# theouterlimitz/Audio-Mastering-Engine

Measured on AMD Instinct MI355X. Metric: mastered Msamples/sec (48 kHz stereo f32) at 1/2/4/8 GPUs; % HBM roofline, higher is better.
Workload: dtype f64

## Files before the change

### audio-mastering-engine_amd/csrc/amx_chain.hip

```cpp
#include "amx_dev.hpp"


namespace amx {

#define AMX_HALF_LUT 32769

__device__ __forceinline__ void decode_in(const ChainDev &cd, const uint32_t *row, int f,
                                          int win, int16_t &l, int16_t &r) {
    if (win == 2) {
        l = q_f32_to_s16_ffmpeg(__uint_as_float(row[2 * f]));
        r = q_f32_to_s16_ffmpeg(__uint_as_float(row[2 * f + 1]));
    } else {
        const uint32_t w = row[f];
        if (cd.in_s16) {
            l = lo16(w);
            r = hi16(w);
        } else {
            l = r = q_f32_to_s16_ffmpeg(__uint_as_float(w));
        }
    }
}

template <int D, int WIN, bool AN, bool SC = false>
__global__ void __launch_bounds__(AMX_BLOCK) k_front1(const ChainDev *__restrict__ cdp,
// ... 335 lines not shown
#pragma unroll
                for (int e = 0; e < 2; e++) {
                    const int qq = (int)q_f32_to_s16_ffmpeg(src[e]);
                    const float v = s_tab[abs(qq)];
                    t2[e] = __int_as_float(__float_as_int(v) | (qq & (int)0x80000000));
                }
                int16_t l, rr;
                analog_shelves(cd, t2[0], t2[1], l, rr);
                a16[q.loc_off + fr] = pack2(l, rr);
            }
        }
    }
}

#define AMX_G16_PITCH (AMX_TF + 4)
template <int D>
__global__ void __launch_bounds__(AMX_BLOCK, 4) k_gemv16(const ChainDev *__restrict__ cdp,
                                                         const ChunkDev *__restrict__ chunks,
                                                         const SegDev *__restrict__ segs,
                                                         int n_seg, int L,
                                                         const uint32_t *__restrict__ a16,
                                                         const double *__restrict__ G,
                                                         double *__restrict__ e) {
    constexpr int ROWS = AMX_BLOCK / 2;
    constexpr int H = D / 2;
    constexpr int GQ = AMX_TF * D / 2;
    static_assert(GQ <= AMX_BLOCK && D % 2 == 0 && D > 0, "tile shape");
    __shared__ __attribute__((aligned(16))) uint32_t s_in[ROWS * AMX_G16_PITCH];
    __shared__ __attribute__((aligned(16))) double sG[AMX_TF * D];
    __shared__ int64_t rb[ROWS];
    __shared__ int rl[ROWS];
// ... 16 lines not shown
    }
    uint4 R[2], RG;
    auto fetch = [&](int k) {
        RG = *reinterpret_cast<const uint4 *>(G + (int64_t)k * D + 2 * (t < GQ ? t : 0));
#pragma unroll
        for (int m = 0; m < 2; m++) {
            const int n = k + c4;
            uint4 v = *reinterpret_cast<const uint4 *>(ip[m] + (n < ilen[m] ? k : 0));
            R[m] = v;
        }
    };
    double a0[H], a1[H];
#pragma unroll
    for (int d = 0; d < H; d++) { a0[d] = 0.0; a1[d] = 0.0; }
    fetch(0);
    const uint32_t *rp = s_in + row * AMX_G16_PITCH;
    for (int k = 0; k < L; k += AMX_TF) {
#pragma unroll
        for (int m = 0; m < 2; m++) {
            uint4 v = R[m];
            const int n = k + c4;
            v.x = n < ilen[m] ? v.x : 0u;
            v.y = n + 1 < ilen[m] ? v.y : 0u;
            v.z = n + 2 < ilen[m] ? v.z : 0u;
            v.w = n + 3 < ilen[m] ? v.w : 0u;
            *reinterpret_cast<uint4 *>(s_in + ((t >> 2) + 64 * m) * AMX_G16_PITCH + c4) = v;
        }
        if (t < GQ) reinterpret_cast<uint4 *>(sG)[t] = RG;
        __syncthreads();
        fetch(k + AMX_TF < L ? k + AMX_TF : k);
#pragma unroll 1
        for (int f = 0; f < AMX_TF; f++) {
            const uint32_t w = rp[f];
            const double x0 = (double)((float)lo16(w) / 32768.0f);
            const double x1 = (double)((float)hi16(w) / 32768.0f);
            const double *g = sG + f * D + half * H;
#pragma unroll
            for (int d = 0; d < H; d++) {
                a0[d] = fma(g[d], x0, a0[d]);
                a1[d] = fma(g[d], x1, a1[d]);
            }
        }
        __syncthreads();
    }
    if (valid && !sg.last) {
        double *eo = e + (int64_t)j * 2 * D + half * H;
#pragma unroll
        for (int d = 0; d < H; d++) { eo[d] = a0[d]; eo[D + d] = a1[d]; }
    }
}
// ... 52 lines not shown
        }
    }
}

__device__ __forceinline__ VRows vt_rows(int32_t base, int len) {
    VRows vr;
    const int r0 = (threadIdx.x & 63) >> 2;
#pragma unroll
    for (int i = 0; i < 2; i++) {
        vr.base[i] = __shfl(base, 2 * (r0 + 16 * i));
        vr.len[i] = __shfl(len, 2 * (r0 + 16 * i));
    }
    return vr;
}

template <int MASK, bool MB, bool KW, bool SC = false>
__global__ void __launch_bounds__(AMX_BLOCK, (MB || KW) ? 4 : 5) k_front2(const ChainDev *__restrict__ cdp,
                                                      const ChunkDev *__restrict__ chunks,
                                                      const SegDev *__restrict__ segs, int n_seg,
                                                      int L, const uint32_t *__restrict__ a16,
                                                      const double *__restrict__ s_eq,
                                                      uint32_t *__restrict__ dst, int to_out,
                                                      const double *__restrict__ Gx,
                                                      double *__restrict__ e_x,
                                                      const double *__restrict__ Gkw,
                                                      double *__restrict__ e_kw,
                                                      uint32_t *__restrict__ pk,
                                                      const float *__restrict__ slut) {
    constexpr int D = EqDim<MASK>::v;
    constexpr int ROWS = AMX_BLOCK / 2;
    constexpr int WV = AMX_BLOCK / 64;
// ... 22 lines not shown
            for (int d = 0; d < D; d++) z[d] = s[d];
        }
    }
    EqState est;
    eq_state_load<MASK>(est, z);
    double xv[MB ? AMX_XO_DIM : 1];
#pragma unroll
    for (int d = 0; d < (MB ? AMX_XO_DIM : 1); d++) xv[d] = 0.0;
    double kv[KW ? AMX_KW_DIM : 1];
#pragma unroll
    for (int d = 0; d < (KW ? AMX_KW_DIM : 1); d++) kv[d] = 0.0;
    int kmax = 0;
    const int klen = (j < n_seg) ? segs[j].len : 0;
    const int negm = (cd.st[0].neg ? 1 : 0) | (cd.st[3].neg ? 8 : 0);
    const float w = cd.width;
    const int won = cd.width_on;
    const VRows vin = vt_rows(b_in, len);
    if (chn == 0) s_orow[wv][row] = make_int2(b_out, len);
    uint32_t *s_in = s_in_all[wv], *s_out = s_out_all[wv];
    vt4 R[2];
    vt_fetch(R, a16, vin, 0);
    for (int k = 0; k < L; k += AMX_TF) {
        vt_put(s_in, R, vin, k);
        amx_wave_sync();
        vt_next(R, a16, vin, k, L);
        const uint32_t *rp = s_in + row * AMX_VT_PITCH;
        uint32_t *op = s_out + row * AMX_VT_PITCH;
#pragma unroll 1
        for (int f0 = 0; f0 < AMX_TF; f0 += AMX_EQ_F) {
            float xf[AMX_EQ_F];
            double x[AMX_EQ_F];
#pragma unroll
            for (int f = 0; f < AMX_EQ_F; f++) {
                const uint32_t p = rp[f0 + f];
                const int16_t sv = chn ? hi16(p) : lo16(p);
                if constexpr (SC) xf[f] = slut ? slut[(int)sv + 32768] : (float)sv / 32768.0f;
                else xf[f] = (float)sv / 32768.0f;
                x[f] = (double)xf[f];
            }
            eq_tile<MASK, AMX_EQ_F>(negm, cd.eqc + (f0 & cd.pad0_), est, x, xf);
#pragma unroll
            for (int f = 0; f < AMX_EQ_F; f++) {
                int16_t qv;
                if constexpr (SC) {
                    qv = MASK ? f64_to_s16(x[f]) : f32_to_s16(xf[f]);
                } else {
                    float v = MASK ? (float)x[f] : xf[f];
                    if (won) {
                        const float o = pair_swap(v);
                        v = width_one(w, chn ? o : v, chn ? v : o, chn);
                    }
                    qv = f32_to_s16(v);
                }
                const int other = __builtin_amdgcn_update_dpp(0, (int)qv, 0xB1, 0xF, 0xF, false);
                if (chn == 0) op[f0 + f] = pack2(qv, (int16_t)other);
                if constexpr (MB) {
                    const double *g = Gx + (int64_t)(k + f0 + f) * AMX_XO_DIM;
                    const double xd = (double)((float)qv / 32768.0f);
#pragma unroll
                    for (int d = 0; d < AMX_XO_DIM; d++) xv[d] = fma(g[d], xd, xv[d]);
                }
                if constexpr (KW) {
                    const int n = k + f0 + f;
                    const bool act = n < klen;
                    kmax = max(kmax, act ? abs((int)qv) : 0);
                    const double xs = act ? (double)qv * (1.0 / 32768.0) : 0.0;
                    const double *g = Gkw + (int64_t)n * AMX_KW_DIM;
#pragma unroll
                    for (int d = 0; d < AMX_KW_DIM; d++) kv[d] = fma(g[d], xs, kv[d]);
                }
            }
        }
        amx_wave_sync();
        {
            const int r0 = (t & 63) >> 2;
            const int2 o0 = s_orow[wv][r0], o1 = s_orow[wv][r0 + 16];
            VRows vout;
            vout.base[0] = o0.x; vout.len[0] = o0.y;
            vout.base[1] = o1.x; vout.len[1] = o1.y;
            vt_store(s_out, dst, vout, k);
        }
// ... 53 lines not shown
#pragma unroll
    for (int sc = 0; sc < 4; sc++) {
        c[5 * sc + 0] = s_c[6 * sc + 0];
        c[5 * sc + 1] = s_c[6 * sc + 1];
        c[5 * sc + 2] = s_c[6 * sc + 2];
        c[5 * sc + 3] = s_c[6 * sc + 4];
        c[5 * sc + 4] = s_c[6 * sc + 5];
    }
    uint32_t *si = s_in[wv], *slo = s_b[wv][0], *smi = s_b[wv][1], *shi = si;
    vt4 R[2];
    vt_fetch(R, p16, vr, 0);
    for (int k = 0; k < L; k += AMX_TF) {
        vt_put(si, R, vr, k);
        amx_wave_sync();
        vt_next(R, p16, vr, k, L);
        uint32_t xin[AMX_TF];
#pragma unroll
        for (int q = 0; q < AMX_TF / 4; q++) {
            const vt4 v = *reinterpret_cast<const vt4 *>(si + row * AMX_VT_PITCH + 4 * q);
            xin[4 * q] = v.x; xin[4 * q + 1] = v.y; xin[4 * q + 2] = v.z; xin[4 * q + 3] = v.w;
        }
        const int o = row * AMX_VT_PITCH;
#pragma unroll 4
        for (int f = 0; f < AMX_TF; f++) {
            const uint32_t p = xin[f];
            const int16_t v = chn ? hi16(p) : lo16(p);
            const double x = (double)((float)v / 32768.0f);
            double l = bq_step(c, z[0], z[1], x);
            l = bq_step(c + 5, z[2], z[3], l);
            double h = bq_step(c + 10, z[4], z[5], x);
            h = bq_step(c + 15, z[6], z[7], h);
            const double m = (x - l) - h;
            const int ql = f64_to_s16(l), qm = f64_to_s16(m), qh = f64_to_s16(h);
            const int ol = __builtin_amdgcn_update_dpp(0, ql, 0xB1, 0xF, 0xF, false);
            const int om = __builtin_amdgcn_update_dpp(0, qm, 0xB1, 0xF, 0xF, false);
            const int oh = __builtin_amdgcn_update_dpp(0, qh, 0xB1, 0xF, 0xF, false);
            if (chn == 0) {
                slo[o + f] = pack2((int16_t)ql, (int16_t)ol);
                smi[o + f] = pack2((int16_t)qm, (int16_t)om);
            } else {
                shi[o + f] = pack2((int16_t)oh, (int16_t)qh);
            }
        }
        amx_wave_sync();
        vt_store(slo, bands, vr, k);
        vt_store(smi, bands + nloc, vr, k);
        vt_store(shi, bands + 2 * nloc, vr, k);
        amx_wave_sync();
    }
}

template <int D, int WIN, bool AN, bool SC = false>
static hipError_t front1_t(const Launch &l, const uint32_t *in, const float *lut, uint32_t *a16,
                           const double *G, double *e) {
    hipLaunchKernelGGL((k_front1<D, WIN, AN, SC>), grid1(l.n_seg), dim3(AMX_BLOCK), 0, l.stream, l.cd,
                       l.chunks, l.segs, l.n_seg, l.L, in, lut, a16, G, e);
// ... 15 lines not shown
static hipError_t front1s_t(const Launch &l, const uint32_t *in, const float *lut, uint32_t *a16,
                            const double *G, double *e) {
    const int rows = AMX_BLOCK / 2;
    if constexpr (AN) {
        if (l.f1_mode == AMX_F1_SPLIT && l.lut_half) {
            const int64_t wgs = l.an_blocks;
            const dim3 gh((unsigned)(wgs < cu_count() ? (wgs > 0 ? wgs : 1) : cu_count()));
            const bool vec = l.an_vec && (reinterpret_cast<uintptr_t>(in) & 15) == 0;
            if (vec)
                hipLaunchKernelGGL(k_analog_h<true>, gh, dim3(1024), 0, l.stream, l.cd, l.chunks, l.n_chunks,
                                   reinterpret_cast<const float *>(in), l.lut_half, a16, l.an_blocks);
            else
                hipLaunchKernelGGL(k_analog_h<false>, gh, dim3(1024), 0, l.stream, l.cd, l.chunks, l.n_chunks,
                                   reinterpret_cast<const float *>(in), l.lut_half, a16, l.an_blocks);
            if constexpr (D > 0) {
                hipLaunchKernelGGL((k_gemv16<D>), dim3((unsigned)((l.n_seg + rows - 1) / rows)), dim3(AMX_BLOCK), 0,
                                   l.stream, l.cd, l.chunks, l.segs, l.n_seg, l.L, a16, G, e);
            }
            return hipGetLastError();
        }
    }
    dim3 grid((unsigned)((l.n_seg + rows - 1) / rows));
    hipLaunchKernelGGL((k_front1s<D, AN>), grid, dim3(AMX_BLOCK), 0, l.stream, l.cd, l.chunks,
                       l.segs, l.n_seg, l.L, in, lut, a16, G, e);
    return hipGetLastError();
}

template <int D, int WIN>
static hipError_t front1_an(const Launch &l, bool an, const uint32_t *in, const float *lut,
                            uint32_t *a16, const double *G, double *e) {
    if constexpr (WIN == 2) {
        if (l.L % AMX_TF) return hipErrorInvalidValue;
// ... 9 lines not shown
    if (l.n_seg <= 0) return hipSuccess;
    if (analog && !lut) return hipErrorInvalidValue;
    if (sc && (analog || win != 1)) return hipErrorInvalidValue;
    const uint32_t *i32 = reinterpret_cast<const uint32_t *>(in);
    uint32_t *a = reinterpret_cast<uint32_t *>(a16);
#define F1(DD)                                                                   \
    case DD:                                                                     \
        if (sc) return front1_t<DD, 1, false, true>(l, i32, lut, a, G, e);       \
        return win == 2 ? front1_an<DD, 2>(l, analog, i32, lut, a, G, e)         \
                        : front1_an<DD, 1>(l, analog, i32, lut, a, G, e);
    switch (D) { F1(0) F1(2) F1(4) F1(8) F1(10) F1(12) F1(16) F1(18) F1(20) }
#undef F1
    return hipErrorInvalidValue;
}

template <int MASK, bool MB, bool KW, bool SC = false>
static hipError_t front2_t(const Launch &l, const uint32_t *a16, const double *s_eq,
                           uint32_t *dst, int to_out, const double *Gx, double *e_x,
                           const double *Gkw, double *e_kw, uint32_t *pk, const float *slut = nullptr) {
    const int rows = AMX_BLOCK / 2;
    dim3 grid((unsigned)((l.n_seg + rows - 1) / rows));
    hipLaunchKernelGGL((k_front2<MASK, MB, KW, SC>), grid, dim3(AMX_BLOCK), 0, l.stream, l.cd,
                       l.chunks, l.segs, l.n_seg, l.L, a16, s_eq, dst, to_out, Gx, e_x, Gkw, e_kw,
                       pk, slut);
    return hipGetLastError();
}

#define AMX_MASK_CASES(X) X(0) X(1) X(2) X(3) X(4) X(5) X(6) X(7) X(8) X(9) X(10) X(11) X(12) X(13) X(14) X(15)

hipError_t launch_front2(const Launch &l, int mask, const int16_t *a16, const double *s_eq,
                         int16_t *dst, int to_out, const double *Gx, double *e_x,
                         const double *Gkw, double *e_kw, uint32_t *pk, bool sc, const float *slut) {
    if (l.n_seg <= 0) return hipSuccess;
    const uint32_t *a = reinterpret_cast<const uint32_t *>(a16);
    uint32_t *d = reinterpret_cast<uint32_t *>(dst);
    const bool mb = Gx != nullptr, kw = Gkw != nullptr;
    if (mb && kw) return hipErrorInvalidValue;
    if (sc && kw) return hipErrorInvalidValue;
    switch (mask) {
#define C2(M)                                                                           \
    case M:                                                                             \
        if (sc) return mb ? front2_t<M, true, false, true>(l, a, s_eq, d, to_out, Gx, e_x, Gkw, e_kw, pk, slut) \
                          : front2_t<M, false, false, true>(l, a, s_eq, d, to_out, Gx, e_x, Gkw, e_kw, pk, slut); \
        return mb ? front2_t<M, true, false>(l, a, s_eq, d, to_out, Gx, e_x, Gkw, e_kw, pk) \
             : kw ? front2_t<M, false, true>(l, a, s_eq, d, to_out, Gx, e_x, Gkw, e_kw, pk) \
                  : front2_t<M, false, false>(l, a, s_eq, d, to_out, Gx, e_x, Gkw, e_kw, pk);
        AMX_MASK_CASES(C2)
#undef C2
    }
    return hipErrorInvalidValue;
}

hipError_t launch_xover2(const Launch &l, const int16_t *p16, const double *s_x,
                         int16_t *bands, int64_t nloc, int *bact) {
    if (l.n_seg <= 0) return hipSuccess;
    const int rows = AMX_BLOCK / 2;
    dim3 grid((unsigned)((l.n_seg + rows - 1) / rows));
    hipLaunchKernelGGL(k_xover2, grid, dim3(AMX_BLOCK), 0, l.stream, l.cd, l.chunks, l.segs,
                       l.n_seg, l.L, reinterpret_cast<const uint32_t *>(p16), s_x,
// ... 6 lines not shown
```

### audio-mastering-engine_amd/csrc/amx_dev.hpp

```cpp
#pragma once
#include "amx_internal.hpp"
#include <math.h>

namespace amx {

__device__ __forceinline__ int16_t q_f32_to_s16_ffmpeg(float x) {
    float v = rintf(x * 32768.0f);
    v = fminf(fmaxf(v, -32768.0f), 32767.0f);
    return (int16_t)(int)v;
}
__device__ __forceinline__ int16_t f32_to_s16(float x) {
    const float v = __builtin_amdgcn_fmed3f(x, -1.0f, 1.0f) * 32767.0f;
    return (int16_t)(int)v;
}
__device__ __forceinline__ double f64_clip1_raw(double x);
__device__ __forceinline__ int16_t f64_to_s16(double x) {
    return (int16_t)(int)(f64_clip1_raw(x) * 32767.0);
}
__device__ __forceinline__ double round2(double v) {
    if (!isfinite(v)) return v;
    const double p = v * 100.0;
    const double err = fma(v, 100.0, -p);
    double k = rint(p);
    if (fabs(p - k) == 0.5 && err != 0.0) k = err > 0.0 ? floor(p) + 1.0 : floor(p);
    return k / 100.0;
}
__device__ __forceinline__ int16_t sat16(int v) {
    return (int16_t)(v > 32767 ? 32767 : (v < -32768 ? -32768 : v));
}
__device__ __forceinline__ uint32_t pack2(int16_t a, int16_t b) {
    return (uint32_t)(uint16_t)a | ((uint32_t)(uint16_t)b << 16);
}
// ... 131 lines not shown
#pragma unroll
        for (int i = 0; i < 8; i++) st.pa[i] = z[o + i];
        o += 8;
    }
    if constexpr ((MASK & 4) != 0) {
#pragma unroll
        for (int i = 0; i < 8; i++) {
            if constexpr ((MASK & 2) != 0) st.pb[i] = z[o + i];
            else st.pa[i] = z[o + i];
        }
        o += 8;
    }
    if constexpr ((MASK & 8) != 0) { st.s3[0] = z[o]; st.s3[1] = z[o + 1]; }
}

template <int MASK, int F>
__device__ __forceinline__ void eq_tile(int negm, const double *__restrict__ sq, EqState &st,
                                        double *x, const float *xf) {
    constexpr int NP = ((MASK >> 1) & 1) + ((MASK >> 2) & 1);
    int c = 0;
    if constexpr ((MASK & 1) != 0) {
        double q[6];
#pragma unroll
        for (int i = 0; i < 6; i++) q[i] = sq[i];
        if (!(negm & 1)) {
#pragma unroll
            for (int f = 0; f < F; f++) {
                const double y = bq_step(q, st.s0[0], st.s0[1], x[f]);
                x[f] = x[f] + (y - x[f]) * q[5];
            }
        } else {
#pragma unroll
            for (int f = 0; f < F; f++) {
                const double y = bq_step(q, st.s0[0], st.s0[1], x[f]);
                const double xg = (double)(xf[f] * (float)q[5]);
                x[f] = xg + (y - xg);
            }
        }
        c = 6;
    }
    if constexpr (NP > 0) {
#pragma unroll 1
        for (int sidx = 0; sidx < NP; sidx++) {
            const double *q = sq + c + 21 * sidx;
            double b[F];
#pragma unroll
            for (int f = 0; f < F; f++) b[f] = x[f];
#pragma unroll
            for (int k = 0; k < 4; k++)
#pragma unroll
                for (int f = 0; f < F; f++)
                    b[f] = bq_step(q + 5 * k, st.pa[2 * k], st.pa[2 * k + 1], b[f]);
            const double gm1 = q[20];
#pragma unroll
            for (int f = 0; f < F; f++) x[f] = x[f] + b[f] * gm1;
            if constexpr (NP == 2) {
#pragma unroll
                for (int i = 0; i < 8; i++) { const double tmp = st.pa[i]; st.pa[i] = st.pb[i]; st.pb[i] = tmp; }
            }
        }
        c += 21 * NP;
    }
    if constexpr ((MASK & 8) != 0) {
        double q[6];
#pragma unroll
        for (int i = 0; i < 6; i++) q[i] = sq[c + i];
        if (!(negm & 8)) {
#pragma unroll
            for (int f = 0; f < F; f++) {
                const double y = bq_step(q, st.s3[0], st.s3[1], x[f]);
                x[f] = x[f] + (y - x[f]) * q[5];
            }
        } else {
#pragma unroll
// ... 6 lines not shown
                    const double xg = x[f] * q[5];
                    x[f] = xg + (y - xg);
                }
            }
        }
    }
}

__device__ __forceinline__ void width_frame(float w, float &l, float &r) {
    float mid = (l + r) / 2.0f, side = (l - r) / 2.0f;
    side = side * w;
    float nl = mid + side, nr = mid - side;
    l = __builtin_amdgcn_fmed3f(nl, -1.0f, 1.0f);
    r = __builtin_amdgcn_fmed3f(nr, -1.0f, 1.0f);
}
__device__ __forceinline__ float width_one(float w, float l, float r, int chn) {
    const float mid = (l + r) / 2.0f, side = ((l - r) / 2.0f) * w;
    return __builtin_amdgcn_fmed3f(chn ? mid - side : mid + side, -1.0f, 1.0f);
}

#define AMX_TF AMX_TF_FRAMES
template <int W, int ROWS = AMX_BLOCK>
struct Tile {
    static constexpr int ROW = AMX_TF * W;
    static constexpr int PITCH = ROW + 1;
    static constexpr int WORDS = ROWS * PITCH;
    static constexpr int ITER = ROWS * ROW / AMX_BLOCK;
    static constexpr int RSTEP = AMX_BLOCK / ROW;
    static constexpr int RW = ROWS / (AMX_BLOCK / 64);
};

template <int W, int ROWS, bool LOCAL>
__device__ __forceinline__ int tile_row(int m) {
// ... 75 lines not shown
__device__ __forceinline__ void tile_store(const uint32_t *lds, uint32_t *__restrict__ dst,
                                           const int64_t *rb, const int *hi, int k) {
    using T = Tile<W, ROWS>;
    const int c = threadIdx.x % T::ROW;
    const int n = k + c / W;
#pragma unroll
    for (int m = 0; m < T::ITER; m++) {
        const int r = tile_row<W, ROWS, LOCAL>(m);
        if (n < hi[r]) dst[rb[r] + (int64_t)n * W + (c % W)] = lds[r * T::PITCH + c];
    }
}

__device__ __forceinline__ float pair_swap(float v) {
    return __int_as_float(__builtin_amdgcn_update_dpp(0, __float_as_int(v), 0xB1, 0xF, 0xF, false));
}
__device__ __forceinline__ double pair_swap(double v) {
    const int64_t b = __double_as_longlong(v);
    const int lo = __builtin_amdgcn_update_dpp(0, (int)(b & 0xffffffff), 0xB1, 0xF, 0xF, false);
    const int hi = __builtin_amdgcn_update_dpp(0, (int)(b >> 32), 0xB1, 0xF, 0xF, false);
    return __longlong_as_double(((int64_t)hi << 32) | (uint32_t)lo);
}

static inline dim3 grid1(int64_t n) { return dim3((unsigned)((n + AMX_BLOCK - 1) / AMX_BLOCK)); }
static inline bool empty(dim3 g) { return g.x == 0 || g.y == 0 || g.z == 0; }

}
```

### audio-mastering-engine_amd/csrc/amx_dyn.hip

```cpp
#include "amx_dev.hpp"

namespace amx {

typedef double d2v __attribute__((ext_vector_type(2)));
typedef uint32_t u4v __attribute__((ext_vector_type(4)));

#define AMX_TAB 32769

#define AMX_RMS_N 4096
#define AMX_RMS_MAXLOOK 1024

__device__ __forceinline__ int rms_slot(int k) { return k + (k >> 4); }

__device__ __forceinline__ uint32_t rms_floor(uint64_t S, uint32_t cnt, double rc) {
    const double sd = fma((double)(uint32_t)(S >> 32), 4294967296.0, (double)(uint32_t)S);
    const double cd = (double)cnt;
    const uint32_t k = (uint32_t)__builtin_amdgcn_sqrtf((float)(sd * rc));
    const uint32_t k1 = k + 1;
    const bool up = (double)__umul24(k1, k1) * cd <= sd;
    const bool down = (double)__umul24(k, k) * cd > sd;
    const uint32_t r = k + (uint32_t)up - (uint32_t)(down & !up);
    return cnt ? (r > 32768u ? 32768u : r) : 0u;
}

// ... 356 lines not shown
    const uint16_t *irow[4];
#pragma unroll
    for (int i = 0; i < 4; i++) {
        const int r = 16 * i + (lane >> 2);
        irow[i] = mi + __shfl(rowoff + start, r) + 4 * (lane & 3);
    }
    u2v I[AMX_ENV_PF][4];
#pragma unroll
    for (int u = 0; u < AMX_ENV_PF; u++)
#pragma unroll
        for (int i = 0; i < 4; i++) I[u][i] = *reinterpret_cast<const u2v *>(irow[i] + u * AMX_ENV_TF);
    double G[2][16];
    env_gather(mt, I[0], G[0]);
    env_gather(mt, I[1], G[1]);
    double att = 0.0, s_spec = 0.0;
    if (cd.env_guess && start >= 0) att = mt[mi[rowoff + start]];
    bool any = false;
    for (int q0 = 0; q0 < ntile; q0 += AMX_ENV_PF) {
#pragma unroll
        for (int u = 0; u < AMX_ENV_PF; u++)
            env0_tile<RCP>(cd, sm, G[u & 1], I[u], I[(u + 2) % AMX_ENV_PF], irow, mt,
                           q0 + u, ntile, nwarm, start, end, ckr, att, s_spec, any);
    }
    if (valid) {
        sv[(int64_t)b * ld + j] = s_spec;
        ev[(int64_t)b * ld + j] = att;
        act[(int64_t)b * ld + j] = any ? 1 : 0;
    }
}

template <bool RCP>
// ... 673 lines not shown
```

### audio-mastering-engine_amd/csrc/amx_internal.hpp

```cpp
#pragma once
#include <hip/hip_runtime.h>
#include <stdint.h>

#include "amx_tables.hpp"

#define AMX_BLOCK 256
#define AMX_HIST_BINS 1000
#define AMX_SCAN_PW 6
#define AMX_CTL_FAST 1
#define AMX_STATS 16
#ifndef AMX_PCM_U8
#define AMX_PCM_U8 0
#define AMX_PCM_S16 1
#define AMX_PCM_S24 2
#define AMX_PCM_S32 3
#define AMX_PCM_F32 4
#define AMX_PCM_F64 5
#define AMX_PCM_S8 6
#define AMX_PCM_S16BE 7
#define AMX_PCM_S24BE 8
#define AMX_PCM_S32BE 9
#define AMX_PCM_F32BE 10
#define AMX_PCM_F64BE 11
#endif

struct amx_flac_cand_t;

namespace amx {
struct Launch {
    const ChainDev *cd;
    const ChunkDev *chunks;
    const SegDev *segs;
    int32_t n_chunks, n_seg, L;
    hipStream_t stream;
    const float *lut_half = nullptr;
    int f1_mode = AMX_F1_SPLIT;
    int64_t max_chunk_n = 0;
    int64_t an_blocks = 0;
    int an_vec = 0;
};
struct ScanPlan {
    int D, n_blk, K;
    const ScanBlk *blks;
    const double *M;
    const double *Mbk;
};
hipError_t launch_front1(const Launch &l, int D, int win, bool analog, const float *in,
                         const float *lut, int16_t *a16, const double *G, double *e, bool sc = false);
hipError_t launch_scan(const ScanPlan &p, const double *e, double *s, const double *carry,
                       double *eb, hipStream_t st, bool up = true, const double *tailP = nullptr,
                       double *tail = nullptr);
hipError_t launch_front2(const Launch &l, int mask, const int16_t *a16, const double *s_eq,
                         int16_t *dst, int to_out, const double *Gx, double *e_x,
                         const double *Gkw, double *e_kw, uint32_t *pk, bool sc = false,
// ... 211 lines not shown
```

### audio-mastering-engine_amd/csrc/amx_plan.cpp

```cpp
#include "../../include/amx.h"
#include "amx_internal.hpp"
#include "amx_plan.hpp"

#include <algorithm>
#include <climits>
#include <cmath>
#include <cstdio>
#include <cstdarg>
#include <cstdlib>
#include <cstring>
#include <memory>
#include <string>
#include <vector>

namespace {

thread_local std::string g_err;

int fail(int code, const char *fmt, ...) {
    char buf[512];
    va_list ap;
    va_start(ap, fmt);
    vsnprintf(buf, sizeof buf, fmt, ap);
    va_end(ap);
// ... 193 lines not shown
    const SpanDev &s = p->spans[track];
    span->out_offset = s.out_off;
    span->out_frames = s.out_n;
    span->track_frame0 = s.tframe0;
    span->track_frames_total = s.ttotal;
    return AMX_OK;
}

int amx_run_stage(amx_plan *p, int32_t stage, const float *d_in, int16_t *d_out, void *d_ws,
                  void *stream) {
    if (!p || (p->nloc > 0 && (!d_in || !d_out || !d_ws))) return fail(AMX_EINVAL, "null argument");
    if (stage < 0 || stage >= AMX_STAGE_COUNT) return fail(AMX_EINVAL, "bad stage %d", stage);
    if (p->n_seg == 0) return AMX_OK;
    hipStream_t st = (hipStream_t)stream;
    amx::Launch l{p->d_cd, p->d_chunks, p->d_segs, p->n_chunks, p->n_seg, p->L, st, p->d_lut_half,
                  p->f1_mode, p->max_chunk_n, p->an_blocks, p->an_vec};
    int16_t *a16 = wsp<int16_t>(d_ws, p->o_a16);
    double *e = wsp<double>(d_ws, p->o_e), *s = wsp<double>(d_ws, p->o_s);
    int16_t *p16 = p->mb ? wsp<int16_t>(d_ws, p->o_p16) : nullptr;
    double *ex = p->mb ? wsp<double>(d_ws, p->o_ex) : nullptr;
    double *sx = p->mb ? wsp<double>(d_ws, p->o_sx) : nullptr;
    int16_t *bands = p->mb ? wsp<int16_t>(d_ws, p->o_bands) : nullptr;
    double *ck = p->mb ? wsp<double>(d_ws, p->o_gain) : nullptr;
    uint16_t *mframe = p->mb ? wsp<uint16_t>(d_ws, p->o_m) : nullptr;
    double *esv = p->mb ? wsp<double>(d_ws, p->o_esv) : nullptr;
    double *ee0 = p->mb ? wsp<double>(d_ws, p->o_ee0) : nullptr;
    int *eflags = p->mb ? wsp<int>(d_ws, p->o_eflags) : nullptr;
    int *eact = p->mb ? wsp<int>(d_ws, p->o_eact) : nullptr;
    int *ehead = p->mb ? wsp<int>(d_ws, p->o_ehead) : nullptr;
    int *elist = p->mb ? wsp<int>(d_ws, p->o_elist) : nullptr;
    int *eprev = p->mb ? wsp<int>(d_ws, p->o_eprev) : nullptr;
// ... 1097 lines not shown
```

### audio-mastering-engine_amd/csrc/amx_plan_build.cpp

```cpp
#include "amx_plan_build.hpp"

#include <climits>
#include <cmath>
#include <cstdarg>
#include <cstdio>
#include <cstdlib>
#include <cstring>

namespace amx {
namespace {

using LD = long double;

MatL matmul(const MatL &a, const MatL &b, int D) {
    MatL c((size_t)D * D, 0.0L);
    for (int i = 0; i < D; i++)
        for (int k = 0; k < D; k++) {
            const LD v = a[(size_t)i * D + k];
            if (v == 0.0L) continue;
            for (int j = 0; j < D; j++) c[(size_t)i * D + j] += v * b[(size_t)k * D + j];
        }
    return c;
}
MatL matpow(const MatL &a, int64_t p, int D) {
// ... 44 lines not shown
        ScanBlk b{};
        b.seg0 = j0 + q;
        b.nseg = (n - q) < AMX_SCAN_S ? (n - q) : AMX_SCAN_S;
        b.first = first;
        b.last = (q + AMX_SCAN_S >= n) ? 1 : 0;
        b.stream = stream;
        out.push_back(b);
    }
}

int64_t overlay_len(int64_t n, int fs) {
    double ms = std::nearbyint(1000.0 * ((double)n / (double)fs));
    return (int64_t)(ms * (fs / 1000.0));
}

}

Mat Lti::pow(int64_t p) const { return to_double(matpow(A, p, D)); }
std::vector<double> Lti::gemv_table(int L) const {
    std::vector<double> G((size_t)L * D);
    std::vector<LD> v = B, t(D);
    for (int n = L - 1; n >= 0; n--) {
        for (int d = 0; d < D; d++) G[(size_t)n * D + d] = (double)v[d];
        for (int i = 0; i < D; i++) {
            LD acc = 0.0L;
            for (int k = 0; k < D; k++) acc += A[(size_t)i * D + k] * v[k];
            t[i] = acc;
        }
        v = t;
    }
// ... 363 lines not shown
        cd.rq[b] = rq;
    }
    {
        static const double exc[16] = {
            0x1.a934f0979a371p+1, -0x1.34413509f79ffp-2, 0x1.9dc1da994fd21p-59,
            -0x1.f48ad494ea3e9p-53, 0x1.26bb1bbb55516p+1, 0x1.ade156a5dcb37p-26,
            0x1.28af3fca7ab0cp-22, 0x1.71dee623fde64p-19, 0x1.a01997c89e6b0p-16,
            0x1.a01a014761f6ep-13, 0x1.6c16c1852b7b0p-10, 0x1.1111111122322p-7,
            0x1.55555555502a1p-5, 0x1.5555555555511p-3, 0x1.000000000000bp-1, 0.05};
        for (int i = 0; i < 16; i++) cd.exc[i] = exc[i];
    }
    cd.env_A = A;
    cd.env_R = R;
    cd.env_rA = 1.0 / A;
    cd.env_rR = 1.0 / R;
    cd.env_guess = 1;
    cd.env_rcp = 1;
    for (size_t i = 0; i < (size_t)3 * 3 * 32769 && cd.env_rcp; i += 1) {
        if (i % (3 * 32769) >= 32769) continue;
        const double m = tabs[i];
        const double qa = m * cd.env_rA, qr = m * cd.env_rR;
        const double ca = std::fma(std::fma(-qa, A, m), cd.env_rA, qa);
        const double cr = std::fma(std::fma(-qr, R, m), cd.env_rR, qr);
        if (ca != m / A || cr != m / R) cd.env_rcp = 0;
    }
    return AMX_OK;
}

int Builder::count_tracks() {
    int n_tracks = 0;
    for (int c = 0; c < n_chunks; c++) {
// ... 264 lines not shown
            return fail(AMX_ERANGE, "EQ decays too slowly for %d-frame segments; raise seg_frames", p->L);
    }
    if (p->mb) {
        Lti xo;
        xo.derive(AMX_XO_DIM, [&](LD *z, LD x) {
            LD l = sos_step_h(cd.xlo, z, x);
            sos_step_h(cd.xlo + 6, z + 2, l);
            LD h = sos_step_h(cd.xhi, z + 4, x);
            sos_step_h(cd.xhi + 6, z + 6, h);
        });
        p->Gx = xo.gemv_table(p->L);
        p->Mx = xo.pow(p->L);
        p->lev_x = xo.window_powers((int64_t)p->L * AMX_SCAN_S, tol, 16, p->Mpx);
        if (p->lev_x < 0) return fail(AMX_ERANGE, "crossover decays too slowly for %d-frame segments", p->L);
    }
    Lti &kw = p->kw_model;
    kw.derive(AMX_KW_DIM, [&](LD *z, LD x) {
        LD y = sos_step_h(cd.kw1, z, x);
        sos_step_h(cd.kw2, z + 2, y);
    });
    const int Lseg = p->resamp ? std::max(1, p->upLout) : p->Lkw;
    if (p->resamp) {
        std::vector<double> &Gkw = p->Gkw, &qh = p->qh, &qt = p->qt;
        LD Cr[AMX_KW_DIM];
        for (int k = 0; k < AMX_KW_DIM; k++) {
            LD z[AMX_KW_DIM] = {0.0L, 0.0L, 0.0L, 0.0L};
            z[k] = 1.0L;
            const LD y1 = sos_step_h(cd.kw1, z, 0.0L);
            Cr[k] = sos_step_h(cd.kw2, z + 2, y1);
        }
// ... 155 lines not shown
```

### audio-mastering-engine_amd/csrc/amx_plan_build.hpp

```cpp
#pragma once
#include "../../include/amx.h"
#include "amx_tables.hpp"

#include <stddef.h>
#include <algorithm>
#include <string>
#include <vector>

namespace amx {

int swr_geometry(int in_rate, int out_rate, int *L, int *M);
int swr_filter(int in_rate, int out_rate, int *taps, int *alloc, double *factor,
               int max_alloc = AMX_SWR_MAX_ALLOC);
int swr_phases(int in_rate, int out_rate, int max_alloc = AMX_SWR_MAX_ALLOC);
int swr_incr(int in_rate, int out_rate, int64_t *src_incr, int64_t *dst_incr);
int swr_bank(int in_rate, int out_rate, float *bank, int max_alloc = AMX_SWR_MAX_ALLOC);

using Mat = std::vector<double>;
using MatL = std::vector<long double>;

struct Lti {
    int D = 0;
    MatL A;
    std::vector<long double> B;
// ... 6 lines not shown
        for (int k = 0; k < D; k++) {
            std::fill(s.begin(), s.end(), 0.0L);
            s[k] = 1.0L;
            step(s.data(), 0.0L);
            for (int i = 0; i < D; i++) A[(size_t)i * D + k] = s[i];
        }
        std::fill(s.begin(), s.end(), 0.0L);
        step(s.data(), 1.0L);
        for (int i = 0; i < D; i++) B[i] = s[i];
    }
    Mat pow(int64_t p) const;
    std::vector<double> gemv_table(int L) const;
    int window_powers(int64_t LS, double tol, int max_k, std::vector<double> &out) const;
};

struct PlanKnobs {
    int up_poly = 1;
    int f1 = AMX_F1_SPLIT;
    static PlanKnobs from_env();
    static bool needs_ncu(bool multiband_on) { return multiband_on; }
};

struct PlanHost {
    amx_chain_desc desc;
    ChainDev cd;
    int L = 256, Lkw = 512, hop = 0;
    int resamp = 0, upL = 1, upM = 1, upLin = 0, upLout = 0, up_static = 0, up_ok = 1;
    int meas_native = 0;
    int up_pc = 1, up_lin = 0;
    int up_taps = 32, up_alloc = 32;
// ... 3 lines not shown
    double kdf_b[5] = {0, 0, 0, 0, 0}, kdf_a[5] = {0, 0, 0, 0, 0};
    int mask = 0, D = 0;
    int lev_eq = 0, lev_x = 0, lev_kw = 0;
    int mb = 0;
    int Le = 1024, warm = 2304, rounds = 2;
    int Le_t[4] = {0, 0, 0, 0};
    int env_wg = 1, env_pin = 0;
    int f1_mode = AMX_F1_SPLIT;
    int n_es = 0;
    int fuse_kw = 0;
    int kw_aligned = 0;
    int n_tracks = 0, n_chunks = 0, n_seg = 0, n_kseg = 0, n_blk = 0, n_kblk = 0;
    int64_t max_nkseg = 0;
    int64_t nloc = 0, out_frames = 0, max_chunk_out = 0, max_span = 0, max_chunk_n = 0;
    int64_t an_blocks = 0;
    int an_vec = 1;
    int64_t in_frames = 0;
    int64_t max_hops = 1;
    int mono16 = 0;
    int sc = 0;
    int any_empty_span = 0;
    std::vector<ChunkDev> chunks;
    std::vector<KwSegDev> ksegs;
    std::vector<SpanDev> spans;
    Lti kw_model;
    std::vector<double> tail_pow;
    std::vector<SegDev> segs, esegs;
    std::vector<int> eseg0, neseg;
    std::vector<ScanBlk> blks, kblks;
    std::vector<int64_t> n1tab;
// ... 19 lines not shown
```

### audio-mastering-engine_amd/csrc/amx_tables.hpp

```cpp
#pragma once
#include <stdint.h>

#define AMX_MAX_EQ_DIM 20
#define AMX_XO_DIM 8
#define AMX_KW_DIM 4
#define AMX_TF_FRAMES 16
#define AMX_SCAN_S 16
#define AMX_ENV_MAX_ROUNDS 16
#define AMX_ENV_NCTR 4
#define AMX_ENV_BACT (AMX_ENV_MAX_ROUNDS * (1 + AMX_ENV_NCTR))
#define AMX_ENV_LIST (AMX_ENV_BACT + 4)
#define AMX_EQC 64
#define AMX_MEAS_RATE 192000
#define AMX_SWR_MAX_ALLOC 144
#define AMX_RS_MAX_ALLOC 256
#define AMX_RS_TILE 256
#define AMX_F1_SPLIT 0
#define AMX_F1_FULL 2

struct EqStageDev {
    int32_t kind;
    int32_t neg;
    double g;
    double gm1;
// ... 11 lines not shown
    float width, drive;
    double an_lo[6];
    double an_glo1;
    double an_hi[6];
    double an_ghi1;
    EqStageDev st[4];
    double xlo[12], xhi[12];
    int32_t look;
    int32_t rthr[3];
    int32_t rq[3];
    int32_t pad_rq_;
    double kw1[6], kw2[6];
    double eqc[AMX_EQC];
    double env_A, env_R, env_rA, env_rR;
    int32_t env_rcp;
    int32_t env_guess;
    int32_t es_ld;
    struct { int32_t es_off, n_es, ch_off, Le; } etab[4];
    double exc[16];
};

struct ChunkDev {
    int64_t in_off;
    int64_t loc_off;
    int64_t out_off;
    int64_t n;
    int64_t out_n;
    int32_t seg0, nseg;
    int32_t track, pad_;
};

// ... 49 lines not shown
```

Before: 30930.

## Fold 1/32768 input scaling into GEMV weights and streamline per-sample int16 paths

Adds a plan-time check that pre-multiplies the crossover weight table by 2^-15 and, when safe, has the gemv16 and front2 kernels use raw int16 samples as doubles, dropping a float divide and convert per sample. It also reads int16 lanes directly from shared memory instead of unpacking 32-bit words, splits the peaking-EQ loop into two scheduled calls with sched barriers and no state swap, replaces the stereo width computation with DPP add-based lane math, and uses perm-based packing. The env_guess flag is removed so the envelope initial guess is always taken. The mixed changes add template variants and depend on the scaling being exact for nonzero weights.

```diff
diff --git a/audio-mastering-engine_amd/csrc/amx_chain.hip b/audio-mastering-engine_amd/csrc/amx_chain.hip
--- a/audio-mastering-engine_amd/csrc/amx_chain.hip
+++ b/audio-mastering-engine_amd/csrc/amx_chain.hip
@@ -373,7 +373,7 @@
 }
 
 #define AMX_G16_PITCH (AMX_TF + 4)
-template <int D>
+template <int D, bool GS>
 __global__ void __launch_bounds__(AMX_BLOCK, 4) k_gemv16(const ChainDev *__restrict__ cdp,
                                                          const ChunkDev *__restrict__ chunks,
                                                          const SegDev *__restrict__ segs,
@@ -420,7 +420,7 @@
 #pragma unroll
     for (int d = 0; d < H; d++) { a0[d] = 0.0; a1[d] = 0.0; }
     fetch(0);
-    const uint32_t *rp = s_in + row * AMX_G16_PITCH;
+    const int16_t *rp = reinterpret_cast<const int16_t *>(s_in + row * AMX_G16_PITCH);
     for (int k = 0; k < L; k += AMX_TF) {
 #pragma unroll
         for (int m = 0; m < 2; m++) {
@@ -432,14 +432,18 @@
             v.w = n + 3 < ilen[m] ? v.w : 0u;
             *reinterpret_cast<uint4 *>(s_in + ((t >> 2) + 64 * m) * AMX_G16_PITCH + c4) = v;
         }
-        if (t < GQ) reinterpret_cast<uint4 *>(sG)[t] = RG;
+        if (t < GQ) {
+            double2 gq = *reinterpret_cast<const double2 *>(&RG);
+            if constexpr (GS) { gq.x *= 0x1p-15; gq.y *= 0x1p-15; }
+            reinterpret_cast<double2 *>(sG)[t] = gq;
+        }
         __syncthreads();
         fetch(k + AMX_TF < L ? k + AMX_TF : k);
 #pragma unroll 1
         for (int f = 0; f < AMX_TF; f++) {
-            const uint32_t w = rp[f];
-            const double x0 = (double)((float)lo16(w) / 32768.0f);
-            const double x1 = (double)((float)hi16(w) / 32768.0f);
+            const int q0 = rp[2 * f], q1 = rp[2 * f + 1];
+            const double x0 = GS ? (double)q0 : (double)((float)q0 / 32768.0f);
+            const double x1 = GS ? (double)q1 : (double)((float)q1 / 32768.0f);
             const double *g = sG + f * D + half * H;
 #pragma unroll
             for (int d = 0; d < H; d++) {
@@ -522,7 +526,7 @@
     return vr;
 }
 
-template <int MASK, bool MB, bool KW, bool SC = false>
+template <int MASK, bool MB, bool KW, bool SC = false, bool GS = false>
 __global__ void __launch_bounds__(AMX_BLOCK, (MB || KW) ? 4 : 5) k_front2(const ChainDev *__restrict__ cdp,
                                                       const ChunkDev *__restrict__ chunks,
                                                       const SegDev *__restrict__ segs, int n_seg,
@@ -575,7 +579,7 @@
     const int klen = (j < n_seg) ? segs[j].len : 0;
     const int negm = (cd.st[0].neg ? 1 : 0) | (cd.st[3].neg ? 8 : 0);
     const float w = cd.width;
-    const int won = cd.width_on;
+    const bool won = !SC && cd.width_on;
     const VRows vin = vt_rows(b_in, len);
     if (chn == 0) s_orow[wv][row] = make_int2(b_out, len);
     uint32_t *s_in = s_in_all[wv], *s_out = s_out_all[wv];
@@ -585,7 +589,7 @@
         vt_put(s_in, R, vin, k);
         amx_wave_sync();
         vt_next(R, a16, vin, k, L);
-        const uint32_t *rp = s_in + row * AMX_VT_PITCH;
+        const int16_t *rp = reinterpret_cast<const int16_t *>(s_in + row * AMX_VT_PITCH) + chn;
         uint32_t *op = s_out + row * AMX_VT_PITCH;
 #pragma unroll 1
         for (int f0 = 0; f0 < AMX_TF; f0 += AMX_EQ_F) {
@@ -593,39 +597,39 @@
             double x[AMX_EQ_F];
 #pragma unroll
             for (int f = 0; f < AMX_EQ_F; f++) {
-                const uint32_t p = rp[f0 + f];
-                const int16_t sv = chn ? hi16(p) : lo16(p);
-                if constexpr (SC) xf[f] = slut ? slut[(int)sv + 32768] : (float)sv / 32768.0f;
-                else xf[f] = (float)sv / 32768.0f;
-                x[f] = (double)xf[f];
-            }
-            eq_tile<MASK, AMX_EQ_F>(negm, cd.eqc + (f0 & cd.pad0_), est, x, xf);
+                const int sv = rp[2 * (f0 + f)];
+                if constexpr (SC) {
+                    xf[f] = slut ? slut[sv + 32768] : (float)sv / 32768.0f;
+                    x[f] = (double)xf[f];
+                } else {
+                    xf[f] = (float)sv / 32768.0f;
+                    x[f] = (double)sv * 0x1p-15;
+                }
+            }
+            eq_tile<MASK, AMX_EQ_F>(negm, cd.eqc + (f0 & cd.pad0_), cd.eqc + ((f0 + 1) & cd.pad0_), est, x, xf);
 #pragma unroll
             for (int f = 0; f < AMX_EQ_F; f++) {
-                int16_t qv;
+                int q;
                 if constexpr (SC) {
-                    qv = MASK ? f64_to_s16(x[f]) : f32_to_s16(xf[f]);
+                    q = MASK ? f64_to_q16(x[f]) : f32_to_q16(xf[f]);
                 } else {
                     float v = MASK ? (float)x[f] : xf[f];
-                    if (won) {
-                        const float o = pair_swap(v);
-                        v = width_one(w, chn ? o : v, chn ? v : o, chn);
-                    }
-                    qv = f32_to_s16(v);
+                    if (won) v = width_lane(w, chn, v);
+                    q = f32_to_q16(v);
                 }
-                const int other = __builtin_amdgcn_update_dpp(0, (int)qv, 0xB1, 0xF, 0xF, false);
-                if (chn == 0) op[f0 + f] = pack2(qv, (int16_t)other);
+                const int other = pair_other(q);
+                if (chn == 0) op[f0 + f] = pack2_lo(q, other);
                 if constexpr (MB) {
                     const double *g = Gx + (int64_t)(k + f0 + f) * AMX_XO_DIM;
-                    const double xd = (double)((float)qv / 32768.0f);
+                    const double xd = GS ? (double)q : (double)((float)q / 32768.0f);
 #pragma unroll
                     for (int d = 0; d < AMX_XO_DIM; d++) xv[d] = fma(g[d], xd, xv[d]);
                 }
                 if constexpr (KW) {
                     const int n = k + f0 + f;
                     const bool act = n < klen;
-                    kmax = max(kmax, act ? abs((int)qv) : 0);
-                    const double xs = act ? (double)qv * (1.0 / 32768.0) : 0.0;
+                    kmax = max(kmax, act ? abs(q) : 0);
+                    const double xs = act ? (double)q * (1.0 / 32768.0) : 0.0;
                     const double *g = Gkw + (int64_t)n * AMX_KW_DIM;
 #pragma unroll
                     for (int d = 0; d < AMX_KW_DIM; d++) kv[d] = fma(g[d], xs, kv[d]);
@@ -709,32 +713,26 @@
         vt_put(si, R, vr, k);
         amx_wave_sync();
         vt_next(R, p16, vr, k, L);
-        uint32_t xin[AMX_TF];
-#pragma unroll
-        for (int q = 0; q < AMX_TF / 4; q++) {
-            const vt4 v = *reinterpret_cast<const vt4 *>(si + row * AMX_VT_PITCH + 4 * q);
-            xin[4 * q] = v.x; xin[4 * q + 1] = v.y; xin[4 * q + 2] = v.z; xin[4 * q + 3] = v.w;
-        }
+        int xin[AMX_TF];
+#pragma unroll
+        for (int f = 0; f < AMX_TF; f++)
+            xin[f] = reinterpret_cast<const int16_t *>(si + row * AMX_VT_PITCH)[2 * f + chn];
         const int o = row * AMX_VT_PITCH;
 #pragma unroll 4
         for (int f = 0; f < AMX_TF; f++) {
-            const uint32_t p = xin[f];
-            const int16_t v = chn ? hi16(p) : lo16(p);
-            const double x = (double)((float)v / 32768.0f);
+            const double x = (double)xin[f] * 0x1p-15;
             double l = bq_step(c, z[0], z[1], x);
             l = bq_step(c + 5, z[2], z[3], l);
             double h = bq_step(c + 10, z[4], z[5], x);
             h = bq_step(c + 15, z[6], z[7], h);
             const double m = (x - l) - h;
-            const int ql = f64_to_s16(l), qm = f64_to_s16(m), qh = f64_to_s16(h);
-            const int ol = __builtin_amdgcn_update_dpp(0, ql, 0xB1, 0xF, 0xF, false);
-            const int om = __builtin_amdgcn_update_dpp(0, qm, 0xB1, 0xF, 0xF, false);
-            const int oh = __builtin_amdgcn_update_dpp(0, qh, 0xB1, 0xF, 0xF, false);
+            const int ql = f64_to_q16(l), qm = f64_to_q16(m), qh = f64_to_q16(h);
+            const int ol = pair_other(ql), om = pair_other(qm), oh = pair_other(qh);
             if (chn == 0) {
-                slo[o + f] = pack2((int16_t)ql, (int16_t)ol);
-                smi[o + f] = pack2((int16_t)qm, (int16_t)om);
+                slo[o + f] = pack2_lo(ql, ol);
+                smi[o + f] = pack2_lo(qm, om);
             } else {
-                shi[o + f] = pack2((int16_t)oh, (int16_t)qh);
+                shi[o + f] = pack2_lo(oh, qh);
             }
         }
         amx_wave_sync();
@@ -780,8 +778,13 @@
                 hipLaunchKernelGGL(k_analog_h<false>, gh, dim3(1024), 0, l.stream, l.cd, l.chunks, l.n_chunks,
                                    reinterpret_cast<const float *>(in), l.lut_half, a16, l.an_blocks);
             if constexpr (D > 0) {
-                hipLaunchKernelGGL((k_gemv16<D>), dim3((unsigned)((l.n_seg + rows - 1) / rows)), dim3(AMX_BLOCK), 0,
-                                   l.stream, l.cd, l.chunks, l.segs, l.n_seg, l.L, a16, G, e);
+                const dim3 gg((unsigned)((l.n_seg + rows - 1) / rows));
+                if (l.gin_scaled)
+                    hipLaunchKernelGGL((k_gemv16<D, true>), gg, dim3(AMX_BLOCK), 0, l.stream, l.cd, l.chunks,
+                                       l.segs, l.n_seg, l.L, a16, G, e);
+                else
+                    hipLaunchKernelGGL((k_gemv16<D, false>), gg, dim3(AMX_BLOCK), 0, l.stream, l.cd, l.chunks,
+                                       l.segs, l.n_seg, l.L, a16, G, e);
             }
             return hipGetLastError();
         }
@@ -821,13 +824,13 @@
     return hipErrorInvalidValue;
 }
 
-template <int MASK, bool MB, bool KW, bool SC = false>
+template <int MASK, bool MB, bool KW, bool SC = false, bool GS = false>
 static hipError_t front2_t(const Launch &l, const uint32_t *a16, const double *s_eq,
                            uint32_t *dst, int to_out, const double *Gx, double *e_x,
                            const double *Gkw, double *e_kw, uint32_t *pk, const float *slut = nullptr) {
     const int rows = AMX_BLOCK / 2;
     dim3 grid((unsigned)((l.n_seg + rows - 1) / rows));
-    hipLaunchKernelGGL((k_front2<MASK, MB, KW, SC>), grid, dim3(AMX_BLOCK), 0, l.stream, l.cd,
+    hipLaunchKernelGGL((k_front2<MASK, MB, KW, SC, GS>), grid, dim3(AMX_BLOCK), 0, l.stream, l.cd,
                        l.chunks, l.segs, l.n_seg, l.L, a16, s_eq, dst, to_out, Gx, e_x, Gkw, e_kw,
                        pk, slut);
     return hipGetLastError();
@@ -841,15 +844,17 @@
     if (l.n_seg <= 0) return hipSuccess;
     const uint32_t *a = reinterpret_cast<const uint32_t *>(a16);
     uint32_t *d = reinterpret_cast<uint32_t *>(dst);
-    const bool mb = Gx != nullptr, kw = Gkw != nullptr;
+    const bool mb = Gx != nullptr, kw = Gkw != nullptr, gs = l.gin_scaled != 0;
     if (mb && kw) return hipErrorInvalidValue;
     if (sc && kw) return hipErrorInvalidValue;
     switch (mask) {
 #define C2(M)                                                                           \
     case M:                                                                             \
-        if (sc) return mb ? front2_t<M, true, false, true>(l, a, s_eq, d, to_out, Gx, e_x, Gkw, e_kw, pk, slut) \
+        if (sc) return mb && gs ? front2_t<M, true, false, true, true>(l, a, s_eq, d, to_out, Gx, e_x, Gkw, e_kw, pk, slut) \
+                     : mb ? front2_t<M, true, false, true>(l, a, s_eq, d, to_out, Gx, e_x, Gkw, e_kw, pk, slut) \
                           : front2_t<M, false, false, true>(l, a, s_eq, d, to_out, Gx, e_x, Gkw, e_kw, pk, slut); \
-        return mb ? front2_t<M, true, false>(l, a, s_eq, d, to_out, Gx, e_x, Gkw, e_kw, pk) \
+        return mb && gs ? front2_t<M, true, false, false, true>(l, a, s_eq, d, to_out, Gx, e_x, Gkw, e_kw, pk) \
+             : mb ? front2_t<M, true, false>(l, a, s_eq, d, to_out, Gx, e_x, Gkw, e_kw, pk) \
              : kw ? front2_t<M, false, true>(l, a, s_eq, d, to_out, Gx, e_x, Gkw, e_kw, pk) \
                   : front2_t<M, false, false>(l, a, s_eq, d, to_out, Gx, e_x, Gkw, e_kw, pk);
         AMX_MASK_CASES(C2)
diff --git a/audio-mastering-engine_amd/csrc/amx_dev.hpp b/audio-mastering-engine_amd/csrc/amx_dev.hpp
--- a/audio-mastering-engine_amd/csrc/amx_dev.hpp
+++ b/audio-mastering-engine_amd/csrc/amx_dev.hpp
@@ -16,6 +16,15 @@
 __device__ __forceinline__ double f64_clip1_raw(double x);
 __device__ __forceinline__ int16_t f64_to_s16(double x) {
     return (int16_t)(int)(f64_clip1_raw(x) * 32767.0);
+}
+__device__ __forceinline__ int f32_to_q16(float x) {
+    return (int)(__builtin_amdgcn_fmed3f(x, -1.0f, 1.0f) * 32767.0f);
+}
+__device__ __forceinline__ int f64_to_q16(double x) {
+    return (int)(f64_clip1_raw(x) * 32767.0);
+}
+__device__ __forceinline__ uint32_t pack2_lo(int a, int b) {
+    return __builtin_amdgcn_perm((uint32_t)b, (uint32_t)a, 0x05040100u);
 }
 __device__ __forceinline__ double round2(double v) {
     if (!isfinite(v)) return v;
@@ -177,9 +186,27 @@
     if constexpr ((MASK & 8) != 0) { st.s3[0] = z[o]; st.s3[1] = z[o + 1]; }
 }
 
+template <int F>
+__device__ __forceinline__ void eq_peak(const double *__restrict__ q, double *pz, double *x) {
+    double b[F];
+#pragma unroll
+    for (int f = 0; f < F; f++) b[f] = x[f];
+#pragma unroll
+    for (int k = 0; k < 4; k++)
+#pragma unroll
+        for (int f = 0; f < F; f++)
+            b[f] = bq_step(q + 5 * k, pz[2 * k], pz[2 * k + 1], b[f]);
+    const double gm1 = q[20];
+#pragma unroll
+    for (int f = 0; f < F; f++) x[f] = x[f] + b[f] * gm1;
+#pragma unroll
+    for (int i = 0; i < 8; i++) asm volatile("" : "+v"(pz[i]));
+}
+
 template <int MASK, int F>
-__device__ __forceinline__ void eq_tile(int negm, const double *__restrict__ sq, EqState &st,
-                                        double *x, const float *xf) {
+__device__ __forceinline__ void eq_tile(int negm, const double *__restrict__ sq,
+                                        const double *__restrict__ sq2, EqState &st, double *x,
+                                        const float *xf) {
     constexpr int NP = ((MASK >> 1) & 1) + ((MASK >> 2) & 1);
     int c = 0;
     if constexpr ((MASK & 1) != 0) {
@@ -203,24 +230,12 @@
         c = 6;
     }
     if constexpr (NP > 0) {
-#pragma unroll 1
-        for (int sidx = 0; sidx < NP; sidx++) {
-            const double *q = sq + c + 21 * sidx;
-            double b[F];
-#pragma unroll
-            for (int f = 0; f < F; f++) b[f] = x[f];
-#pragma unroll
-            for (int k = 0; k < 4; k++)
-#pragma unroll
-                for (int f = 0; f < F; f++)
-                    b[f] = bq_step(q + 5 * k, st.pa[2 * k], st.pa[2 * k + 1], b[f]);
-            const double gm1 = q[20];
-#pragma unroll
-            for (int f = 0; f < F; f++) x[f] = x[f] + b[f] * gm1;
-            if constexpr (NP == 2) {
-#pragma unroll
-                for (int i = 0; i < 8; i++) { const double tmp = st.pa[i]; st.pa[i] = st.pb[i]; st.pb[i] = tmp; }
-            }
+        __builtin_amdgcn_sched_barrier(0);
+        eq_peak<F>(sq + c, st.pa, x);
+        __builtin_amdgcn_sched_barrier(0);
+        if constexpr (NP == 2) {
+            eq_peak<F>(sq2 + c + 21, st.pb, x);
+            __builtin_amdgcn_sched_barrier(0);
         }
         c += 21 * NP;
     }
@@ -257,9 +272,25 @@
     l = __builtin_amdgcn_fmed3f(nl, -1.0f, 1.0f);
     r = __builtin_amdgcn_fmed3f(nr, -1.0f, 1.0f);
 }
-__device__ __forceinline__ float width_one(float w, float l, float r, int chn) {
-    const float mid = (l + r) / 2.0f, side = ((l - r) / 2.0f) * w;
-    return __builtin_amdgcn_fmed3f(chn ? mid - side : mid + side, -1.0f, 1.0f);
+__device__ __forceinline__ float width_sign(float v, int chn) {
+    return chn ? -v : v;
+}
+__device__ __forceinline__ float width_mix(float w, int chn, float sum, float dif) {
+    const float mid = sum / 2.0f, side = (dif / 2.0f) * w;
+    return mid + width_sign(side, chn);
+}
+__device__ __forceinline__ float width_self(float w, int chn, float a, float b, float ea, float eb) {
+    return width_mix(w, chn, a + b, ea + eb);
+}
+__device__ __forceinline__ float pair_add(float a, float x) {
+    float r;
+    asm("s_nop 1\n\tv_add_f32_dpp %0, %1, %2 quad_perm:[1,0,3,2] row_mask:0xf bank_mask:0xf bound_ctrl:1"
+        : "=v"(r) : "v"(x), "v"(a));
+    return r;
+}
+__device__ __forceinline__ float width_lane(float w, int chn, float a) {
+    const float e = width_sign(a, chn);
+    return width_mix(w, chn, pair_add(a, a), pair_add(e, e));
 }
 
 #define AMX_TF AMX_TF_FRAMES
@@ -365,6 +396,12 @@
 __device__ __forceinline__ float pair_swap(float v) {
     return __int_as_float(__builtin_amdgcn_update_dpp(0, __float_as_int(v), 0xB1, 0xF, 0xF, false));
 }
+__device__ __forceinline__ int pair_other(int v) {
+    return __builtin_amdgcn_mov_dpp(v, 0xB1, 0xF, 0xF, true);
+}
+__device__ __forceinline__ float pair_other(float v) {
+    return __int_as_float(pair_other(__float_as_int(v)));
+}
 __device__ __forceinline__ double pair_swap(double v) {
     const int64_t b = __double_as_longlong(v);
     const int lo = __builtin_amdgcn_update_dpp(0, (int)(b & 0xffffffff), 0xB1, 0xF, 0xF, false);
diff --git a/audio-mastering-engine_amd/csrc/amx_dyn.hip b/audio-mastering-engine_amd/csrc/amx_dyn.hip
--- a/audio-mastering-engine_amd/csrc/amx_dyn.hip
+++ b/audio-mastering-engine_amd/csrc/amx_dyn.hip
@@ -394,7 +394,7 @@
     env_gather(mt, I[0], G[0]);
     env_gather(mt, I[1], G[1]);
     double att = 0.0, s_spec = 0.0;
-    if (cd.env_guess && start >= 0) att = mt[mi[rowoff + start]];
+    if (start >= 0) att = mt[mi[rowoff + start]];
     bool any = false;
     for (int q0 = 0; q0 < ntile; q0 += AMX_ENV_PF) {
 #pragma unroll
diff --git a/audio-mastering-engine_amd/csrc/amx_internal.hpp b/audio-mastering-engine_amd/csrc/amx_internal.hpp
--- a/audio-mastering-engine_amd/csrc/amx_internal.hpp
+++ b/audio-mastering-engine_amd/csrc/amx_internal.hpp
@@ -38,6 +38,7 @@
     int64_t max_chunk_n = 0;
     int64_t an_blocks = 0;
     int an_vec = 0;
+    int gin_scaled = 0;
 };
 struct ScanPlan {
     int D, n_blk, K;
diff --git a/audio-mastering-engine_amd/csrc/amx_plan.cpp b/audio-mastering-engine_amd/csrc/amx_plan.cpp
--- a/audio-mastering-engine_amd/csrc/amx_plan.cpp
+++ b/audio-mastering-engine_amd/csrc/amx_plan.cpp
@@ -231,7 +231,7 @@
     if (p->n_seg == 0) return AMX_OK;
     hipStream_t st = (hipStream_t)stream;
     amx::Launch l{p->d_cd, p->d_chunks, p->d_segs, p->n_chunks, p->n_seg, p->L, st, p->d_lut_half,
-                  p->f1_mode, p->max_chunk_n, p->an_blocks, p->an_vec};
+                  p->f1_mode, p->max_chunk_n, p->an_blocks, p->an_vec, p->gin_scaled};
     int16_t *a16 = wsp<int16_t>(d_ws, p->o_a16);
     double *e = wsp<double>(d_ws, p->o_e), *s = wsp<double>(d_ws, p->o_s);
     int16_t *p16 = p->mb ? wsp<int16_t>(d_ws, p->o_p16) : nullptr;
diff --git a/audio-mastering-engine_amd/csrc/amx_plan_build.cpp b/audio-mastering-engine_amd/csrc/amx_plan_build.cpp
--- a/audio-mastering-engine_amd/csrc/amx_plan_build.cpp
+++ b/audio-mastering-engine_amd/csrc/amx_plan_build.cpp
@@ -82,6 +82,14 @@
     return (int64_t)(ms * (fs / 1000.0));
 }
 
+}
+
+bool scale_gemv_rows(const std::vector<double> &G, std::vector<double> &Gx) {
+    for (const std::vector<double> *t : {&G, static_cast<const std::vector<double> *>(&Gx)})
+        for (double g : *t)
+            if (!(g == 0.0 || std::fabs(g) >= 0x1p-1007)) return false;
+    for (double &g : Gx) g *= 0x1p-15;
+    return true;
 }
 
 Mat Lti::pow(int64_t p) const { return to_double(matpow(A, p, D)); }
@@ -475,7 +483,6 @@
     cd.env_R = R;
     cd.env_rA = 1.0 / A;
     cd.env_rR = 1.0 / R;
-    cd.env_guess = 1;
     cd.env_rcp = 1;
     for (size_t i = 0; i < (size_t)3 * 3 * 32769 && cd.env_rcp; i += 1) {
         if (i % (3 * 32769) >= 32769) continue;
@@ -770,6 +777,7 @@
         p->lev_x = xo.window_powers((int64_t)p->L * AMX_SCAN_S, tol, 16, p->Mpx);
         if (p->lev_x < 0) return fail(AMX_ERANGE, "crossover decays too slowly for %d-frame segments", p->L);
     }
+    p->gin_scaled = scale_gemv_rows(p->G, p->Gx) ? 1 : 0;
     Lti &kw = p->kw_model;
     kw.derive(AMX_KW_DIM, [&](LD *z, LD x) {
         LD y = sos_step_h(cd.kw1, z, x);
diff --git a/audio-mastering-engine_amd/csrc/amx_plan_build.hpp b/audio-mastering-engine_amd/csrc/amx_plan_build.hpp
--- a/audio-mastering-engine_amd/csrc/amx_plan_build.hpp
+++ b/audio-mastering-engine_amd/csrc/amx_plan_build.hpp
@@ -44,6 +44,8 @@
     int window_powers(int64_t LS, double tol, int max_k, std::vector<double> &out) const;
 };
 
+bool scale_gemv_rows(const std::vector<double> &G, std::vector<double> &Gx);
+
 struct PlanKnobs {
     int up_poly = 1;
     int f1 = AMX_F1_SPLIT;
@@ -77,6 +79,7 @@
     int64_t max_nkseg = 0;
     int64_t nloc = 0, out_frames = 0, max_chunk_out = 0, max_span = 0, max_chunk_n = 0;
     int64_t an_blocks = 0;
+    int gin_scaled = 0;
     int an_vec = 1;
     int64_t in_frames = 0;
     int64_t max_hops = 1;
diff --git a/audio-mastering-engine_amd/csrc/amx_tables.hpp b/audio-mastering-engine_amd/csrc/amx_tables.hpp
--- a/audio-mastering-engine_amd/csrc/amx_tables.hpp
+++ b/audio-mastering-engine_amd/csrc/amx_tables.hpp
@@ -49,7 +49,7 @@
     double eqc[AMX_EQC];
     double env_A, env_R, env_rA, env_rR;
     int32_t env_rcp;
-    int32_t env_guess;
+    int32_t pad1_;
     int32_t es_ld;
     struct { int32_t es_off, n_es, ch_off, Le; } etab[4];
     double exc[16];
```

Result: faster. 31390 (median of 6 runs) (+1.5%).
